# xuelunshen/gim

Hardware: AMD Instinct MI355X
Metric: image-pairs/sec at 640x480 (higher is better)
Workload: dtype fp16

## Files before the change

### gim_amd/csrc/emit.hip

```cpp
#include "gim_common.h"

namespace {

struct Segs { gim_copy_segs s; };

__global__ void __launch_bounds__(256) copy_segments_kernel(const Segs a) {
    const int k = blockIdx.y;
    const char* src = (const char*)a.s.src[k];
    char* dst = (char*)a.s.dst[k];
    const int64_t n = a.s.bytes[k];
    const int64_t t = (int64_t)blockIdx.x * blockDim.x + threadIdx.x, nt = (int64_t)gridDim.x * blockDim.x;
    const bool vec = (((uintptr_t)src | (uintptr_t)dst) & 15) == 0;
    const int64_t nv = vec ? n >> 4 : 0;
    for (int64_t i = t; i < nv; i += nt) ((uint4*)dst)[i] = src ? ((const uint4*)src)[i] : make_uint4(0u, 0u, 0u, 0u);
    for (int64_t i = (nv << 4) + t; i < n; i += nt) dst[i] = src ? src[i] : (char)0;
}

__global__ void __launch_bounds__(256) pack_matches_kernel(const int64_t* __restrict__ m_bids, const float2* __restrict__ mk0,
                                                           const float2* __restrict__ mk1, const float* __restrict__ conf,
                                                           const int64_t* __restrict__ pair_ids, int64_t pid_base,
                                                           float* __restrict__ out, int M) {
    const int m = blockIdx.x * blockDim.x + threadIdx.x;
    if (m >= M) return;
    const int64_t b = m_bids[m];
    const float pid = (float)(pair_ids ? pair_ids[b] : pid_base + b);
    const float2 p0 = mk0[m], p1 = mk1[m];
    float* o = out + (size_t)m * 6;
    *(float2*)(o + 0) = make_float2(pid, p0.x);
    *(float2*)(o + 2) = make_float2(p0.y, p1.x);
    *(float2*)(o + 4) = make_float2(p1.y, conf[m]);
}

constexpr int TL_THREADS = 1024, TL_MAX_FLAGS = 32768;

template <bool REACH2, bool QUARTER>
__device__ __forceinline__ void fine_tile_list_body(const int64_t* __restrict__ b_ids, const int64_t* __restrict__ i_ids,
                                                    const int64_t* __restrict__ j_ids, const int* __restrict__ count, int cap,
                                                    int bs, int w0c, int w1c, int stride, int H, int W,
                                                    int* __restrict__ tiles, int* __restrict__ n_tiles, int tiles_cap,
                                                    int* __restrict__ tiles2, int* __restrict__ n_tiles2,
                                                    int* __restrict__ tilesq, int* __restrict__ n_tilesq, int tilesq_cap) {
    static_assert(!QUARTER || REACH2, "the quarter-level lists are derived from the +-4 flags");
    __shared__ __attribute__((aligned(16))) unsigned char flags[TL_MAX_FLAGS];
    __shared__ int part[TL_THREADS];
    __shared__ int part2[REACH2 ? TL_THREADS : 1];
    __shared__ int partq[QUARTER ? TL_THREADS : 1][2];
    const int t = threadIdx.x;
    const int tiles_x = (W + 31) / 32, tiles_y = (H + 7) / 8, per_img = tiles_x * tiles_y, nflags = 2 * bs * per_img;
    const int h = H / 2, w = W / 2, qtiles_x = w / 32, qtiles_y = h / 8, qper_img = qtiles_x * qtiles_y;
    const int qbase = (nflags + 3) & ~3, nqflags = QUARTER ? 2 * bs * qper_img : 0;
    for (int i = t; i < (QUARTER ? qbase + nqflags : nflags); i += TL_THREADS) flags[i] = 0;
    __syncthreads();
    int M = count[0];
    M = M < 0 ? 0 : (M < cap ? M : cap);
    for (int m = t; m < M; m += TL_THREADS) {
        const int64_t b = b_ids[m];
        if (b < 0 || b >= bs) continue;
#pragma unroll
        for (int side = 0; side < 2; ++side) {
            const int64_t cell = side ? j_ids[m] : i_ids[m];
            const int wc = side ? w1c : w0c;
            if (cell < 0 || cell >= (int64_t)wc * ((H + stride - 1) / stride)) continue;
            const int cy = (int)cell / wc, cx = (int)cell - cy * wc;
            int y0 = cy * stride - 3, y1 = cy * stride + 3, x0 = cx * stride - 3, x1 = cx * stride + 3;
            y0 = y0 < 0 ? 0 : y0; x0 = x0 < 0 ? 0 : x0;
            y1 = y1 > H - 1 ? H - 1 : y1; x1 = x1 > W - 1 ? W - 1 : x1;
            if (y0 > y1 || x0 > x1) continue;
            const int img = side * bs + (int)b;
            if constexpr (REACH2) {
                int Y0 = cy * stride - 4, Y1 = cy * stride + 4, X0 = cx * stride - 4, X1 = cx * stride + 4;
                Y0 = Y0 < 0 ? 0 : Y0; X0 = X0 < 0 ? 0 : X0;
                Y1 = Y1 > H - 1 ? H - 1 : Y1; X1 = X1 > W - 1 ? W - 1 : X1;
                for (int ty = Y0 >> 3; ty <= (Y1 >> 3); ++ty)
                    for (int tx = X0 >> 5; tx <= (X1 >> 5); ++tx) {
                        const bool in3 = ty >= (y0 >> 3) && ty <= (y1 >> 3) && tx >= (x0 >> 5) && tx <= (x1 >> 5);
                        const int f = (img * tiles_y + ty) * tiles_x + tx;
                        atomicOr((unsigned*)flags + (f >> 2), (in3 ? 3u : 2u) << (8 * (f & 3)));
                    }
            } else {
            for (int ty = y0 >> 3; ty <= (y1 >> 3); ++ty)
                for (int tx = x0 >> 5; tx <= (x1 >> 5); ++tx) flags[(img * tiles_y + ty) * tiles_x + tx] = 1;
            }
        }
    }
    __syncthreads();
    if constexpr (QUARTER) {
        unsigned char* const qf = flags + qbase;
        const float sy = (float)(h - 1) / (float)(H - 1), sx = (float)(w - 1) / (float)(W - 1);
        for (int i = t; i < nflags; i += TL_THREADS) {
            if (!(flags[i] & 2)) continue;
            const int img = i / per_img, r = i - img * per_img, ty = r / tiles_x, tx = r - ty * tiles_x;
            const int xa = (int)(sx * (32 * tx));
            const int xe = xa + 23 < w - 1 ? xa + 23 : w - 1;
            for (int Y = 8 * ty; Y < 8 * ty + 8 && Y < H; ++Y) {
                const float fy = sy * Y;
                const int y0 = (int)fy, y1 = y0 + (y0 < h - 1 ? 1 : 0);
#pragma unroll
                for (int d = 0; d < 3; ++d) {
                    const int ra = y0 - d > 0 ? y0 - d : 0, rb = y1 + d < h - 1 ? y1 + d : h - 1;
                    const int ca = xa - d > 0 ? xa - d : 0, cb = xe + d < w - 1 ? xe + d : w - 1;
                    const unsigned bits = d == 0 ? 7u : (d == 1 ? 6u : 4u);
                    for (int qy = ra >> 3; qy <= (rb >> 3); ++qy)
                        for (int qx = ca >> 5; qx <= (cb >> 5); ++qx) {
                            const int f = (img * qtiles_y + qy) * qtiles_x + qx;
                            if ((qf[f] & bits) != bits) atomicOr((unsigned*)qf + (f >> 2), bits << (8 * (f & 3)));
                        }
                }
            }
        }
        __syncthreads();
    }
    const int per = (nflags + TL_THREADS - 1) / TL_THREADS;
    const int lo = t * per < nflags ? t * per : nflags, hi = lo + per < nflags ? lo + per : nflags;
    int n = 0, n2 = 0;
    for (int i = lo; i < hi; ++i) { n += flags[i] & 1; n2 += flags[i] >> 1; }
    part[t] = n;
    if constexpr (REACH2) part2[t] = n2;
    const int qper = (nqflags + TL_THREADS - 1) / TL_THREADS;
    const int qlo = t * qper < nqflags ? t * qper : nqflags, qhi = qlo + qper < nqflags ? qlo + qper : nqflags;
    int nab = 0, nc = 0;
    if constexpr (QUARTER) {
        for (int i = qlo; i < qhi; ++i) {
            const int f = flags[qbase + i];
            nab += ((f >> 2) & 1) << 16 | ((f >> 1) & 1);
            nc += f & 1;
        }
        partq[t][0] = nab; partq[t][1] = nc;
    }
    __syncthreads();
    for (int d = 1; d < TL_THREADS; d <<= 1) {
        const int v = t >= d ? part[t - d] : 0;
        const int v2 = REACH2 && t >= d ? part2[t - d] : 0;
        const int vab = QUARTER && t >= d ? partq[t - d][0] : 0, vc = QUARTER && t >= d ? partq[t - d][1] : 0;
        __syncthreads();
        part[t] += v;
        if constexpr (REACH2) part2[t] += v2;
        if constexpr (QUARTER) { partq[t][0] += vab; partq[t][1] += vc; }
        __syncthreads();
    }
    int o = part[t] - n;
    for (int i = lo; i < hi; ++i)
        if (flags[i] & 1) {
            if (o < tiles_cap) tiles[o] = i;
            ++o;
        }
    if (t == TL_THREADS - 1) n_tiles[0] = part[t] < tiles_cap ? part[t] : tiles_cap;
    if constexpr (REACH2) {
        int o2 = part2[t] - n2;
        for (int i = lo; i < hi; ++i)
            if (flags[i] & 2) {
                if (o2 < tiles_cap) tiles2[o2] = i;
                ++o2;
            }
        if (t == TL_THREADS - 1) n_tiles2[0] = part2[t] < tiles_cap ? part2[t] : tiles_cap;
    }
    if constexpr (QUARTER) {
        int oa = (partq[t][0] >> 16) - (nab >> 16), ob = (partq[t][0] & 0xffff) - (nab & 0xffff), oc = partq[t][1] - nc;
        for (int i = qlo; i < qhi; ++i) {
            const int f = flags[qbase + i];
            if (f & 4) { if (oa < tilesq_cap) tilesq[oa] = i; ++oa; }
            if (f & 2) { if (ob < tilesq_cap) tilesq[tilesq_cap + ob] = i; ++ob; }
            if (f & 1) { if (oc < tilesq_cap) tilesq[2 * tilesq_cap + oc] = i; ++oc; }
        }
        if (t == TL_THREADS - 1) {
            const int ta = partq[t][0] >> 16, tb = partq[t][0] & 0xffff, tc = partq[t][1];
            n_tilesq[0] = ta < tilesq_cap ? ta : tilesq_cap;
            n_tilesq[1] = tb < tilesq_cap ? tb : tilesq_cap;
            n_tilesq[2] = tc < tilesq_cap ? tc : tilesq_cap;
        }
    }
}

template <bool REACH2>
__global__ void __launch_bounds__(TL_THREADS) fine_tile_list_kernel(const int64_t* __restrict__ b_ids, const int64_t* __restrict__ i_ids,
                                                                  const int64_t* __restrict__ j_ids, const int* __restrict__ count, int cap,
                                                                  int bs, int w0c, int w1c, int stride, int H, int W,
                                                                  int* __restrict__ tiles, int* __restrict__ n_tiles, int tiles_cap,
                                                                  int* __restrict__ tiles2, int* __restrict__ n_tiles2) {
    fine_tile_list_body<REACH2, false>(b_ids, i_ids, j_ids, count, cap, bs, w0c, w1c, stride, H, W, tiles, n_tiles, tiles_cap, tiles2, n_tiles2,
                                       nullptr, nullptr, 0);
}

__global__ void __launch_bounds__(TL_THREADS) fine_tile_lists4_kernel(const int64_t* __restrict__ b_ids, const int64_t* __restrict__ i_ids,
                                                                    const int64_t* __restrict__ j_ids, const int* __restrict__ count, int cap,
                                                                    int bs, int w0c, int w1c, int stride, int H, int W,
                                                                    int* __restrict__ tiles, int* __restrict__ n_tiles, int tiles_cap,
                                                                    int* __restrict__ tiles2, int* __restrict__ n_tiles2,
                                                                    int* __restrict__ tilesq, int* __restrict__ n_tilesq, int tilesq_cap) {
    fine_tile_list_body<true, true>(b_ids, i_ids, j_ids, count, cap, bs, w0c, w1c, stride, H, W, tiles, n_tiles, tiles_cap, tiles2, n_tiles2,
                                    tilesq, n_tilesq, tilesq_cap);
}

}

extern "C" int gim_fine_tile_list_max_flags(void) { return TL_MAX_FLAGS; }

extern "C" int gim_fine_tile_list(const int64_t* b_ids, const int64_t* i_ids, const int64_t* j_ids, const int* count, int cap, int bs,
                                  int w0c, int w1c, int stride, int H, int W, int* tiles, int* n_tiles, int tiles_cap, gim_stream_t stream) {
    GIM_REQUIRE(b_ids && i_ids && j_ids && count && tiles && n_tiles, "gim_fine_tile_list: NULL pointer");
    GIM_REQUIRE(cap >= 0 && bs > 0 && w0c > 0 && w1c > 0 && stride > 0 && H > 0 && W > 0, "gim_fine_tile_list: bad geometry");
    const int64_t nflags = 2ll * bs * ((W + 31) / 32) * ((H + 7) / 8);
    GIM_REQUIRE(nflags <= TL_MAX_FLAGS, "gim_fine_tile_list: %lld patches exceed the %d flags of the one-workgroup kernel", (long long)nflags, TL_MAX_FLAGS);
    GIM_REQUIRE(tiles_cap >= nflags, "gim_fine_tile_list: the list holds %d entries, the maps have %lld patches", tiles_cap, (long long)nflags);
    hipLaunchKernelGGL(fine_tile_list_kernel<false>, dim3(1), dim3(TL_THREADS), 0, (hipStream_t)stream, b_ids, i_ids, j_ids, count, cap, bs, w0c, w1c,
                       stride, H, W, tiles, n_tiles, tiles_cap, nullptr, nullptr);
    return gim_check_launch("fine_tile_list_kernel");
}

extern "C" int gim_fine_tile_lists(const int64_t* b_ids, const int64_t* i_ids, const int64_t* j_ids, const int* count, int cap, int bs,
                                   int w0c, int w1c, int stride, int H, int W, int* tiles, int* n_tiles, int* tiles4, int* n_tiles4,
                                   int tiles_cap, gim_stream_t stream) {
    GIM_REQUIRE(b_ids && i_ids && j_ids && count && tiles && n_tiles && tiles4 && n_tiles4, "gim_fine_tile_lists: NULL pointer");
    GIM_REQUIRE(cap >= 0 && bs > 0 && w0c > 0 && w1c > 0 && stride > 0 && H > 0 && W > 0, "gim_fine_tile_lists: bad geometry");
    const int64_t nflags = 2ll * bs * ((W + 31) / 32) * ((H + 7) / 8);
    GIM_REQUIRE(nflags <= TL_MAX_FLAGS, "gim_fine_tile_lists: %lld patches exceed the %d flags of the one-workgroup kernel", (long long)nflags, TL_MAX_FLAGS);
    GIM_REQUIRE(tiles_cap >= nflags, "gim_fine_tile_lists: the lists hold %d entries each, the maps have %lld patches", tiles_cap, (long long)nflags);
    hipLaunchKernelGGL(fine_tile_list_kernel<true>, dim3(1), dim3(TL_THREADS), 0, (hipStream_t)stream, b_ids, i_ids, j_ids, count, cap, bs, w0c, w1c,
                       stride, H, W, tiles, n_tiles, tiles_cap, tiles4, n_tiles4);
    return gim_check_launch("fine_tile_list_kernel");
}

extern "C" int gim_fine_tile_lists4(const int64_t* b_ids, const int64_t* i_ids, const int64_t* j_ids, const int* count, int cap, int bs,
                                    int w0c, int w1c, int stride, int H, int W, int* tiles, int* n_tiles, int* tiles4, int* n_tiles4,
                                    int tiles_cap, int* tilesq, int* n_tilesq, int tilesq_cap, gim_stream_t stream) {
    GIM_REQUIRE(b_ids && i_ids && j_ids && count && tiles && n_tiles && tiles4 && n_tiles4 && tilesq && n_tilesq, "gim_fine_tile_lists4: NULL pointer");
    GIM_REQUIRE(cap >= 0 && bs > 0 && w0c > 0 && w1c > 0 && stride > 0 && H > 0 && W > 0, "gim_fine_tile_lists4: bad geometry");
    GIM_REQUIRE(H % 16 == 0 && W % 64 == 0, "gim_fine_tile_lists4: the 1/4-resolution maps (%d x %d) must be whole 8 x 32 patches", H / 2, W / 2);
    const int64_t nflags = 2ll * bs * (W / 32) * (H / 8), nq = 2ll * bs * (W / 64) * (H / 16);
    GIM_REQUIRE(((nflags + 3) & ~3ll) + nq <= TL_MAX_FLAGS, "gim_fine_tile_lists4: %lld + %lld patches exceed the %d flags of the one-workgroup kernel",
                (long long)nflags, (long long)nq, TL_MAX_FLAGS);
    GIM_REQUIRE(tiles_cap >= nflags && tilesq_cap >= nq, "gim_fine_tile_lists4: the lists hold %d / %d entries each, the maps have %lld / %lld patches",
                tiles_cap, tilesq_cap, (long long)nflags, (long long)nq);
    hipLaunchKernelGGL(fine_tile_lists4_kernel, dim3(1), dim3(TL_THREADS), 0, (hipStream_t)stream, b_ids, i_ids, j_ids, count, cap, bs, w0c, w1c,
                       stride, H, W, tiles, n_tiles, tiles_cap, tiles4, n_tiles4, tilesq, n_tilesq, tilesq_cap);
    return gim_check_launch("fine_tile_lists4_kernel");
}

extern "C" int gim_copy_segments(const gim_copy_segs* sp, gim_stream_t stream) {
    GIM_REQUIRE(sp, "gim_copy_segments: NULL args");
    GIM_REQUIRE(sp->n >= 0 && sp->n <= GIM_MAX_COPY_SEGS, "gim_copy_segments: n=%d outside [0, %d]", sp->n, GIM_MAX_COPY_SEGS);
    int64_t mx = 0;
    for (int k = 0; k < sp->n; ++k) {
        GIM_REQUIRE(sp->bytes[k] >= 0 && (sp->bytes[k] == 0 || sp->dst[k]), "gim_copy_segments: segment %d: bad size / NULL dst", k);
        mx = sp->bytes[k] > mx ? sp->bytes[k] : mx;
    }
    if (sp->n == 0 || mx == 0) return GIM_OK;
    Segs a;
    a.s = *sp;
    int64_t blocks = (mx / 16 + 255) / 256;
    blocks = blocks < 1 ? 1 : (blocks > 1024 ? 1024 : blocks);
    hipLaunchKernelGGL(copy_segments_kernel, dim3((unsigned)blocks, (unsigned)sp->n), dim3(256), 0, (hipStream_t)stream, a);
    return gim_check_launch("copy_segments_kernel");
}

extern "C" int gim_pack_matches(const int64_t* m_bids, const float* mkpts0, const float* mkpts1, const float* mconf,
                                const int64_t* pair_ids, int64_t pid_base, float* out, int M, gim_stream_t stream) {
    GIM_REQUIRE(M >= 0, "gim_pack_matches: M=%d", M);
    if (M == 0) return GIM_OK;
    GIM_REQUIRE(m_bids && mkpts0 && mkpts1 && mconf && out, "gim_pack_matches: NULL pointer");
    hipLaunchKernelGGL(pack_matches_kernel, dim3((unsigned)((M + 255) / 256)), dim3(256), 0, (hipStream_t)stream, m_bids,
                       (const float2*)mkpts0, (const float2*)mkpts1, mconf, pair_ids, pid_base, out, M);
    return gim_check_launch("pack_matches_kernel");
}
```

Before: 961.0.

## Split fine tile-list build into multi-block global marking and one-block compaction

The single-workgroup kernel that marked the +-3/+-4 and quarter-resolution tile flags in shared memory is split in two. A grid-wide kernel now marks the flags with global atomics, one thread per match side, and skips the quarter-level marking when a tile was already marked. A one-workgroup kernel then loads the flags, clears them, and runs a wave-shuffle scan to emit the lists. This spreads the serial marking work across the GPU and removes the per-row quarter loop. In exchange it adds a second launch, global atomics, and a persistent per-device workspace that must be allocated outside graph capture.

Result: no change. 966.6, median of 6 (+0.6%).

```diff
diff --git a/gim_amd/csrc/emit.hip b/gim_amd/csrc/emit.hip
--- a/gim_amd/csrc/emit.hip
+++ b/gim_amd/csrc/emit.hip
@@ -1,4 +1,8 @@
 #include "gim_common.h"
+#include <mutex>
+
+GIM_TT_DECL(tile_marks)
+GIM_TT_DECL(tile_lists)
 
 namespace {
 
@@ -33,23 +37,18 @@
 
 constexpr int TL_THREADS = 1024, TL_MAX_FLAGS = 32768;
 
-template <bool REACH2, bool QUARTER>
+template <bool REACH2>
 __device__ __forceinline__ void fine_tile_list_body(const int64_t* __restrict__ b_ids, const int64_t* __restrict__ i_ids,
                                                     const int64_t* __restrict__ j_ids, const int* __restrict__ count, int cap,
                                                     int bs, int w0c, int w1c, int stride, int H, int W,
                                                     int* __restrict__ tiles, int* __restrict__ n_tiles, int tiles_cap,
-                                                    int* __restrict__ tiles2, int* __restrict__ n_tiles2,
-                                                    int* __restrict__ tilesq, int* __restrict__ n_tilesq, int tilesq_cap) {
-    static_assert(!QUARTER || REACH2, "the quarter-level lists are derived from the +-4 flags");
+                                                    int* __restrict__ tiles2, int* __restrict__ n_tiles2) {
     __shared__ __attribute__((aligned(16))) unsigned char flags[TL_MAX_FLAGS];
     __shared__ int part[TL_THREADS];
     __shared__ int part2[REACH2 ? TL_THREADS : 1];
-    __shared__ int partq[QUARTER ? TL_THREADS : 1][2];
     const int t = threadIdx.x;
     const int tiles_x = (W + 31) / 32, tiles_y = (H + 7) / 8, per_img = tiles_x * tiles_y, nflags = 2 * bs * per_img;
-    const int h = H / 2, w = W / 2, qtiles_x = w / 32, qtiles_y = h / 8, qper_img = qtiles_x * qtiles_y;
-    const int qbase = (nflags + 3) & ~3, nqflags = QUARTER ? 2 * bs * qper_img : 0;
-    for (int i = t; i < (QUARTER ? qbase + nqflags : nflags); i += TL_THREADS) flags[i] = 0;
+    for (int i = t; i < nflags; i += TL_THREADS) flags[i] = 0;
     __syncthreads();
     int M = count[0];
     M = M < 0 ? 0 : (M < cap ? M : cap);
@@ -84,58 +83,19 @@
         }
     }
     __syncthreads();
-    if constexpr (QUARTER) {
-        unsigned char* const qf = flags + qbase;
-        const float sy = (float)(h - 1) / (float)(H - 1), sx = (float)(w - 1) / (float)(W - 1);
-        for (int i = t; i < nflags; i += TL_THREADS) {
-            if (!(flags[i] & 2)) continue;
-            const int img = i / per_img, r = i - img * per_img, ty = r / tiles_x, tx = r - ty * tiles_x;
-            const int xa = (int)(sx * (32 * tx));
-            const int xe = xa + 23 < w - 1 ? xa + 23 : w - 1;
-            for (int Y = 8 * ty; Y < 8 * ty + 8 && Y < H; ++Y) {
-                const float fy = sy * Y;
-                const int y0 = (int)fy, y1 = y0 + (y0 < h - 1 ? 1 : 0);
-#pragma unroll
-                for (int d = 0; d < 3; ++d) {
-                    const int ra = y0 - d > 0 ? y0 - d : 0, rb = y1 + d < h - 1 ? y1 + d : h - 1;
-                    const int ca = xa - d > 0 ? xa - d : 0, cb = xe + d < w - 1 ? xe + d : w - 1;
-                    const unsigned bits = d == 0 ? 7u : (d == 1 ? 6u : 4u);
-                    for (int qy = ra >> 3; qy <= (rb >> 3); ++qy)
-                        for (int qx = ca >> 5; qx <= (cb >> 5); ++qx) {
-                            const int f = (img * qtiles_y + qy) * qtiles_x + qx;
-                            if ((qf[f] & bits) != bits) atomicOr((unsigned*)qf + (f >> 2), bits << (8 * (f & 3)));
-                        }
-                }
-            }
-        }
-        __syncthreads();
-    }
     const int per = (nflags + TL_THREADS - 1) / TL_THREADS;
     const int lo = t * per < nflags ? t * per : nflags, hi = lo + per < nflags ? lo + per : nflags;
     int n = 0, n2 = 0;
     for (int i = lo; i < hi; ++i) { n += flags[i] & 1; n2 += flags[i] >> 1; }
     part[t] = n;
     if constexpr (REACH2) part2[t] = n2;
-    const int qper = (nqflags + TL_THREADS - 1) / TL_THREADS;
-    const int qlo = t * qper < nqflags ? t * qper : nqflags, qhi = qlo + qper < nqflags ? qlo + qper : nqflags;
-    int nab = 0, nc = 0;
-    if constexpr (QUARTER) {
-        for (int i = qlo; i < qhi; ++i) {
-            const int f = flags[qbase + i];
-            nab += ((f >> 2) & 1) << 16 | ((f >> 1) & 1);
-            nc += f & 1;
-        }
-        partq[t][0] = nab; partq[t][1] = nc;
-    }
     __syncthreads();
     for (int d = 1; d < TL_THREADS; d <<= 1) {
         const int v = t >= d ? part[t - d] : 0;
         const int v2 = REACH2 && t >= d ? part2[t - d] : 0;
-        const int vab = QUARTER && t >= d ? partq[t - d][0] : 0, vc = QUARTER && t >= d ? partq[t - d][1] : 0;
         __syncthreads();
         part[t] += v;
         if constexpr (REACH2) part2[t] += v2;
-        if constexpr (QUARTER) { partq[t][0] += vab; partq[t][1] += vc; }
         __syncthreads();
     }
     int o = part[t] - n;
@@ -154,21 +114,6 @@
             }
         if (t == TL_THREADS - 1) n_tiles2[0] = part2[t] < tiles_cap ? part2[t] : tiles_cap;
     }
-    if constexpr (QUARTER) {
-        int oa = (partq[t][0] >> 16) - (nab >> 16), ob = (partq[t][0] & 0xffff) - (nab & 0xffff), oc = partq[t][1] - nc;
-        for (int i = qlo; i < qhi; ++i) {
-            const int f = flags[qbase + i];
-            if (f & 4) { if (oa < tilesq_cap) tilesq[oa] = i; ++oa; }
-            if (f & 2) { if (ob < tilesq_cap) tilesq[tilesq_cap + ob] = i; ++ob; }
-            if (f & 1) { if (oc < tilesq_cap) tilesq[2 * tilesq_cap + oc] = i; ++oc; }
-        }
-        if (t == TL_THREADS - 1) {
-            const int ta = partq[t][0] >> 16, tb = partq[t][0] & 0xffff, tc = partq[t][1];
-            n_tilesq[0] = ta < tilesq_cap ? ta : tilesq_cap;
-            n_tilesq[1] = tb < tilesq_cap ? tb : tilesq_cap;
-            n_tilesq[2] = tc < tilesq_cap ? tc : tilesq_cap;
-        }
-    }
 }
 
 template <bool REACH2>
@@ -177,18 +122,158 @@
                                                                   int bs, int w0c, int w1c, int stride, int H, int W,
                                                                   int* __restrict__ tiles, int* __restrict__ n_tiles, int tiles_cap,
                                                                   int* __restrict__ tiles2, int* __restrict__ n_tiles2) {
-    fine_tile_list_body<REACH2, false>(b_ids, i_ids, j_ids, count, cap, bs, w0c, w1c, stride, H, W, tiles, n_tiles, tiles_cap, tiles2, n_tiles2,
-                                       nullptr, nullptr, 0);
-}
-
-__global__ void __launch_bounds__(TL_THREADS) fine_tile_lists4_kernel(const int64_t* __restrict__ b_ids, const int64_t* __restrict__ i_ids,
+    fine_tile_list_body<REACH2>(b_ids, i_ids, j_ids, count, cap, bs, w0c, w1c, stride, H, W, tiles, n_tiles, tiles_cap, tiles2, n_tiles2);
+}
+
+constexpr int TM_THREADS = 256;
+
+__device__ __forceinline__ unsigned tile_mark(unsigned* __restrict__ flags, int f, unsigned bits) {
+    unsigned* const word = flags + (f >> 2);
+    const int sh = 8 * (f & 3);
+    unsigned old = __hip_atomic_load(word, __ATOMIC_RELAXED, __HIP_MEMORY_SCOPE_AGENT);
+    if (((old >> sh) & bits) != bits) old = __hip_atomic_fetch_or(word, bits << sh, __ATOMIC_RELAXED, __HIP_MEMORY_SCOPE_AGENT);
+    return (old >> sh) & 0xffu;
+}
+
+__global__ void __launch_bounds__(TM_THREADS) fine_tile_marks4_kernel(const int64_t* __restrict__ b_ids, const int64_t* __restrict__ i_ids,
                                                                     const int64_t* __restrict__ j_ids, const int* __restrict__ count, int cap,
                                                                     int bs, int w0c, int w1c, int stride, int H, int W,
+                                                                    unsigned* __restrict__ flags) {
+    GIM_TT(tile_marks, 0, 0);
+    const int64_t t = (int64_t)blockIdx.x * TM_THREADS + threadIdx.x;
+    int M = count[0];
+    M = M < 0 ? 0 : (M < cap ? M : cap);
+    if (t >= 2 * (int64_t)M) return;
+    const int m = (int)(t >> 1), side = (int)(t & 1);
+    const int64_t b = b_ids[m];
+    if (b < 0 || b >= bs) return;
+    const int64_t cell = side ? j_ids[m] : i_ids[m];
+    const int wc = side ? w1c : w0c;
+    if (cell < 0 || cell >= (int64_t)wc * ((H + stride - 1) / stride)) return;
+    const int cy = (int)cell / wc, cx = (int)cell - cy * wc;
+    int y0 = cy * stride - 3, y1 = cy * stride + 3, x0 = cx * stride - 3, x1 = cx * stride + 3;
+    y0 = y0 < 0 ? 0 : y0; x0 = x0 < 0 ? 0 : x0;
+    y1 = y1 > H - 1 ? H - 1 : y1; x1 = x1 > W - 1 ? W - 1 : x1;
+    if (y0 > y1 || x0 > x1) return;
+    int Y0 = cy * stride - 4, Y1 = cy * stride + 4, X0 = cx * stride - 4, X1 = cx * stride + 4;
+    Y0 = Y0 < 0 ? 0 : Y0; X0 = X0 < 0 ? 0 : X0;
+    Y1 = Y1 > H - 1 ? H - 1 : Y1; X1 = X1 > W - 1 ? W - 1 : X1;
+    const int tiles_x = W / 32, tiles_y = H / 8, img = side * bs + (int)b;
+    const int h = H / 2, w = W / 2, qtiles_x = w / 32, qtiles_y = h / 8;
+    unsigned* const qflags = flags + (2 * bs * tiles_x * tiles_y + 3) / 4;
+    const float sy = (float)(h - 1) / (float)(H - 1), sx = (float)(w - 1) / (float)(W - 1);
+    for (int ty = Y0 >> 3; ty <= (Y1 >> 3); ++ty)
+        for (int tx = X0 >> 5; tx <= (X1 >> 5); ++tx) {
+            const bool in3 = ty >= (y0 >> 3) && ty <= (y1 >> 3) && tx >= (x0 >> 5) && tx <= (x1 >> 5);
+            if (tile_mark(flags, (img * tiles_y + ty) * tiles_x + tx, in3 ? 3u : 2u) & 2u) continue;
+            const int xa = (int)(sx * (32 * tx));
+            const int xe = xa + 23 < w - 1 ? xa + 23 : w - 1;
+            const int Yl = 8 * ty + 7 < H - 1 ? 8 * ty + 7 : H - 1;
+            const int ya = (int)(sy * (8 * ty)), yl = (int)(sy * Yl), yb = yl + (yl < h - 1 ? 1 : 0);
+#pragma unroll
+            for (int d = 0; d < 3; ++d) {
+                const int ra = ya - d > 0 ? ya - d : 0, rb = yb + d < h - 1 ? yb + d : h - 1;
+                const int ca = xa - d > 0 ? xa - d : 0, cb = xe + d < w - 1 ? xe + d : w - 1;
+                const unsigned bits = d == 0 ? 7u : (d == 1 ? 6u : 4u);
+                for (int qy = ra >> 3; qy <= (rb >> 3); ++qy)
+                    for (int qx = ca >> 5; qx <= (cb >> 5); ++qx) tile_mark(qflags, (img * qtiles_y + qy) * qtiles_x + qx, bits);
+            }
+        }
+    GIM_TT(tile_marks, 0, 1);
+}
+
+__global__ void __launch_bounds__(TL_THREADS) fine_tile_lists4_kernel(unsigned* __restrict__ gflags, int bs, int H, int W,
                                                                     int* __restrict__ tiles, int* __restrict__ n_tiles, int tiles_cap,
                                                                     int* __restrict__ tiles2, int* __restrict__ n_tiles2,
                                                                     int* __restrict__ tilesq, int* __restrict__ n_tilesq, int tilesq_cap) {
-    fine_tile_list_body<true, true>(b_ids, i_ids, j_ids, count, cap, bs, w0c, w1c, stride, H, W, tiles, n_tiles, tiles_cap, tiles2, n_tiles2,
-                                    tilesq, n_tilesq, tilesq_cap);
+    __shared__ __attribute__((aligned(16))) unsigned words[TL_MAX_FLAGS / 4];
+    __shared__ int wave_tot[TL_THREADS / 64][3];
+    const unsigned char* const flags = (const unsigned char*)words;
+    const int t = threadIdx.x, lane = t & 63, wave = t >> 6;
+    const int nflags = 2 * bs * (W / 32) * (H / 8), qbase = (nflags + 3) & ~3, nqflags = 2 * bs * (W / 64) * (H / 16);
+    if (t < 64) GIM_TT(tile_lists, 0, 0);
+    for (int i = t; i < (qbase + nqflags + 3) / 4; i += TL_THREADS) {
+        words[i] = __hip_atomic_load(gflags + i, __ATOMIC_RELAXED, __HIP_MEMORY_SCOPE_AGENT);
+        __hip_atomic_store(gflags + i, 0u, __ATOMIC_RELAXED, __HIP_MEMORY_SCOPE_AGENT);
+    }
+    __syncthreads();
+    if (t < 64) GIM_TT(tile_lists, 0, 1);
+    const int per = (nflags + TL_THREADS - 1) / TL_THREADS;
+    const int lo = t * per < nflags ? t * per : nflags, hi = lo + per < nflags ? lo + per : nflags;
+    const int qper = (nqflags + TL_THREADS - 1) / TL_THREADS;
+    const int qlo = t * qper < nqflags ? t * qper : nqflags, qhi = qlo + qper < nqflags ? qlo + qper : nqflags;
+    int own[3] = {0, 0, 0};
+    for (int i = lo; i < hi; ++i) own[0] += (flags[i] & 2) << 15 | (flags[i] & 1);
+    for (int i = qlo; i < qhi; ++i) {
+        const int f = flags[qbase + i];
+        own[1] += (f & 4) << 14 | ((f >> 1) & 1);
+        own[2] += f & 1;
+    }
+    int inc[3] = {own[0], own[1], own[2]};
+#pragma unroll
+    for (int d = 1; d < 64; d <<= 1)
+#pragma unroll
+        for (int k = 0; k < 3; ++k) {
+            const int v = __shfl_up(inc[k], d, 64);
+            inc[k] += lane >= d ? v : 0;
+        }
+    if (lane == 63)
+        for (int k = 0; k < 3; ++k) wave_tot[wave][k] = inc[k];
+    __syncthreads();
+    int total[3] = {0, 0, 0}, off[3];
+#pragma unroll
+    for (int k = 0; k < 3; ++k) off[k] = inc[k] - own[k];
+    for (int v = 0; v < TL_THREADS / 64; ++v)
+#pragma unroll
+        for (int k = 0; k < 3; ++k) {
+            const int s = wave_tot[v][k];
+            total[k] += s;
+            off[k] += v < wave ? s : 0;
+        }
+    if (t < 64) GIM_TT(tile_lists, 0, 2);
+    int o = off[0] & 0xffff, o2 = off[0] >> 16;
+    for (int i = lo; i < hi; ++i) {
+        const int f = flags[i];
+        if (f & 1) { if (o < tiles_cap) tiles[o] = i; ++o; }
+        if (f & 2) { if (o2 < tiles_cap) tiles2[o2] = i; ++o2; }
+    }
+    int oa = off[1] >> 16, ob = off[1] & 0xffff, oc = off[2];
+    for (int i = qlo; i < qhi; ++i) {
+        const int f = flags[qbase + i];
+        if (f & 4) { if (oa < tilesq_cap) tilesq[oa] = i; ++oa; }
+        if (f & 2) { if (ob < tilesq_cap) tilesq[tilesq_cap + ob] = i; ++ob; }
+        if (f & 1) { if (oc < tilesq_cap) tilesq[2 * tilesq_cap + oc] = i; ++oc; }
+    }
+    if (t == 0) {
+        const int t3 = total[0] & 0xffff, t4 = total[0] >> 16, ta = total[1] >> 16, tb = total[1] & 0xffff, tc = total[2];
+        n_tiles[0] = t3 < tiles_cap ? t3 : tiles_cap;
+        n_tiles2[0] = t4 < tiles_cap ? t4 : tiles_cap;
+        n_tilesq[0] = ta < tilesq_cap ? ta : tilesq_cap;
+        n_tilesq[1] = tb < tilesq_cap ? tb : tilesq_cap;
+        n_tilesq[2] = tc < tilesq_cap ? tc : tilesq_cap;
+    }
+    if (t < 64) GIM_TT(tile_lists, 0, 3);
+}
+
+int tile_flag_words(hipStream_t stream, unsigned** out) {
+    static std::mutex mu;
+    static unsigned* ws[256] = {};
+    const std::lock_guard<std::mutex> lock(mu);
+    unsigned*& p = ws[GimPerDevice::dev()];
+    if (!p) {
+        hipStreamCaptureStatus st = hipStreamCaptureStatusNone;
+        GIM_REQUIRE(hipStreamIsCapturing(stream, &st) == hipSuccess && st == hipStreamCaptureStatusNone,
+                    "gim_fine_tile_lists4: the first call on a device allocates the flag workspace and cannot be captured: call it once outside the capture");
+        void* q = nullptr;
+        GIM_REQUIRE(hipMalloc(&q, TL_MAX_FLAGS) == hipSuccess, "gim_fine_tile_lists4: no memory for the %d-byte flag workspace", TL_MAX_FLAGS);
+        if (hipMemsetAsync(q, 0, TL_MAX_FLAGS, stream) != hipSuccess) {
+            (void)hipFree(q);
+            GIM_REQUIRE(false, "gim_fine_tile_lists4: clearing the flag workspace failed");
+        }
+        p = (unsigned*)q;
+    }
+    *out = p;
+    return GIM_OK;
 }
 
 }
@@ -231,8 +316,14 @@
                 (long long)nflags, (long long)nq, TL_MAX_FLAGS);
     GIM_REQUIRE(tiles_cap >= nflags && tilesq_cap >= nq, "gim_fine_tile_lists4: the lists hold %d / %d entries each, the maps have %lld / %lld patches",
                 tiles_cap, tilesq_cap, (long long)nflags, (long long)nq);
-    hipLaunchKernelGGL(fine_tile_lists4_kernel, dim3(1), dim3(TL_THREADS), 0, (hipStream_t)stream, b_ids, i_ids, j_ids, count, cap, bs, w0c, w1c,
-                       stride, H, W, tiles, n_tiles, tiles_cap, tiles4, n_tiles4, tilesq, n_tilesq, tilesq_cap);
+    unsigned* flags = nullptr;
+    if (const int rc = tile_flag_words((hipStream_t)stream, &flags)) return rc;
+    const int64_t blocks = (2ll * cap + TM_THREADS - 1) / TM_THREADS;
+    hipLaunchKernelGGL(fine_tile_marks4_kernel, dim3((unsigned)(blocks < 1 ? 1 : blocks)), dim3(TM_THREADS), 0, (hipStream_t)stream, b_ids, i_ids,
+                       j_ids, count, cap, bs, w0c, w1c, stride, H, W, flags);
+    if (const int rc = gim_check_launch("fine_tile_marks4_kernel")) return rc;
+    hipLaunchKernelGGL(fine_tile_lists4_kernel, dim3(1), dim3(TL_THREADS), 0, (hipStream_t)stream, flags, bs, H, W, tiles, n_tiles, tiles_cap,
+                       tiles4, n_tiles4, tilesq, n_tilesq, tilesq_cap);
     return gim_check_launch("fine_tile_lists4_kernel");
 }
 
```
